# rrrickyz/Parallel-and-Distributed-Deep-Learning

Hardware: AMD Instinct MI355X
Metric: images/sec ResNet-50/ImageNet at 1/2/4/8 MI355X + scaling efficiency (higher is better)
Workload: dtype bf16; 1 GPU; model=ResNet-50 Keras-v1 (25,636,712 params, random init), global_batch=2560, per_gpu_batch=2560, image_size=224, parallelism=dp1, replicas=1, optimizer=adam, bn=frozen (training=False), hip_graph=False, grad_dtype=fp32, device=MI355X

## Files before the change

### csrc/bindings.cpp

```cpp
#include <torch/extension.h>

#include <atomic>
#include <ATen/hip/HIPContext.h>
#include <ATen/hip/impl/HIPGuardImplMasqueradingAsCUDA.h>
#include <c10/util/Optional.h>

#include "kernels/kernels.h"

using torch::Tensor;
using OptT = c10::optional<Tensor>;
namespace py = pybind11;

#define PCHECK(cond, msg) TORCH_CHECK(cond, "pddl: ", msg)

namespace {

std::atomic<bool> g_launched{false};
std::atomic<bool> g_knob_tuning{false};
hipStream_t cur_stream() {
  if (!g_launched.load(std::memory_order_relaxed)) g_launched.store(true, std::memory_order_relaxed);
  return at::hip::getCurrentHIPStream().stream();
}

void ok(const char* err, const char* what) { TORCH_CHECK(err == nullptr, "pddl ", what, ": ", err ? err : ""); }
// ... 744 lines not shown
  m.def("comm_proxy", [](Tensor src, Tensor scratch, int passes, int64_t ticks, int nch) {
    PCHECK(src.is_cuda() && scratch.is_cuda() && src.scalar_type() == torch::kFloat32 &&
               scratch.scalar_type() == torch::kFloat32 && src.is_contiguous() && scratch.is_contiguous() &&
               scratch.numel() >= src.numel() && src.numel() % 4 == 0,
           "comm_proxy: fp32 device tensors, scratch >= src, 4-element multiple");
    ok(pddl::comm_proxy_launch(f32p(src), f32p(scratch), src.numel(), passes, ticks, nch, cur_stream()),
       "comm_proxy");
  }, REL);
  const py::none none;
  m.def("igemm", &igemm, REL, py::arg("a1"), py::arg("a2") = none, py::arg("H"), py::arg("W"), py::arg("R"),
        py::arg("S"), py::arg("stride"), py::arg("pad"), py::arg("Ho"), py::arg("Wo"), py::arg("b"), py::arg("mode"),
        py::arg("scale") = none, py::arg("shift") = none, py::arg("res") = none, py::arg("mask") = none,
        py::arg("add") = none, py::arg("out"), py::arg("relu") = 0, py::arg("out2") = none, py::arg("relu2") = 0,
        py::arg("n_split") = 0, py::arg("up2") = 0, py::arg("Hf") = 0, py::arg("Wf") = 0, py::arg("colsum") = none,
        py::arg("bits_out") = none, py::arg("stats") = none, py::arg("bn_z") = none, py::arg("bn_mean") = none);
  m.def("bn_stats", &bn_stats, REL);
  m.def("bn_apply", &bn_apply, REL, py::arg("z"), py::arg("a"), py::arg("b"), py::arg("r") = none,
        py::arg("a2") = none, py::arg("b2") = none, py::arg("relu"), py::arg("y"), py::arg("bits") = none);
  m.def("bn_bwd_reduce", &bn_bwd_reduce, REL, py::arg("g"), py::arg("z"), py::arg("z2") = none, py::arg("mean"),
        py::arg("mean2") = none, py::arg("sg"), py::arg("sgx"), py::arg("sg2") = none, py::arg("sgx2") = none);
  m.def("bn_bwd_apply", &bn_bwd_apply, REL, py::arg("g"), py::arg("z"), py::arg("z2") = none, py::arg("l"),
        py::arg("l2") = std::vector<double>{}, py::arg("params"), py::arg("mean"), py::arg("inv"), py::arg("sg"),
        py::arg("sgx"), py::arg("dz"), py::arg("dz2") = none, py::arg("grads"), py::arg("coef"));
  m.attr("BNSTAT_LAYER_BYTES") = (int)sizeof(pddl::BnStatLayer);
  m.def("wgrad", &wgrad, REL, py::arg("x"), py::arg("H"), py::arg("W"), py::arg("R"), py::arg("S"),
        py::arg("stride"), py::arg("pad"), py::arg("Ho"), py::arg("Wo"), py::arg("g"), py::arg("g2") = none,
        py::arg("co_split") = 0, py::arg("dw"), py::arg("K"), py::arg("splits") = 0);
  m.def("bwd1x1", &bwd1x1, REL, py::arg("g"), py::arg("x"), py::arg("wd"), py::arg("bits"), py::arg("out"),
        py::arg("colsum"), py::arg("dw"), py::arg("out2") = py::none(), py::arg("g1") = py::none(),
        py::arg("w1d") = py::none(), py::arg("gmask") = py::none(), py::arg("gx") = py::none(),
        py::arg("colsum_gx") = py::none());
  m.def("bwd1x1_partial_rows", &bwd1x1_partial_rows);
  m.def("conv_f32", &conv_f32, REL);
  m.def("conv_f32_epi", &conv_f32_epi, REL, py::arg("x"), py::arg("R"), py::arg("S"), py::arg("stride"),
        py::arg("pad"), py::arg("Ho"), py::arg("Wo"), py::arg("w"), py::arg("epi"), py::arg("scale") = none,
        py::arg("shift") = none, py::arg("res") = none, py::arg("relu") = 0, py::arg("add") = none,
        py::arg("mask") = none, py::arg("up2") = 0, py::arg("y"), py::arg("colsum") = none);
  m.def("maxpool_fwd_f32", &maxpool_fwd_f32, REL);
  m.def("maxpool_bwd_f32", &maxpool_bwd_f32, REL);
  m.def("gap_fwd_f32", &gap_fwd_f32, REL);
  m.def("gap_bwd_f32", &gap_bwd_f32, REL);
  m.def("colsum_f32", &colsum_f32, REL);
  m.def("softmax_xent_f32", &softmax_xent_f32, REL);
  m.def("prep_f32", &prep_f32, REL);
  m.def("wgrad_f32", &wgrad_f32, REL);
  m.def("stem_s2d", &stem_s2d, REL);
  m.def("stem_wgrad_fold", &stem_wgrad_fold, REL);
  m.def("maxpool_fwd", &maxpool_fwd, REL);
  m.def("stem_pool_bwd", &stem_pool_bwd, REL, py::arg("x2"), py::arg("gpool"), py::arg("idx"), py::arg("dw"),
        py::arg("colsum"), py::arg("pool_rows") = 0);
  m.def("stem_pool_bwd_partial_rows", [](int B, int H2, int PB) { return pddl::stem_pool_bwd_partial_rows(B, H2, PB); },
        py::arg("B"), py::arg("H2"), py::arg("pool_rows") = 0);
  m.def("stem_pool_fwd", &stem_pool_fwd, REL, py::arg("x2"), py::arg("w"), py::arg("scale"), py::arg("shift"),
        py::arg("pool"), py::arg("idx"), py::arg("bits") = py::none(), py::arg("pool_rows") = 0);
  m.def("maxpool_bwd", &maxpool_bwd, REL);
  m.def("conv3x3c64", &conv3x3c64, REL, py::arg("x"), py::arg("w"), py::arg("mode"), py::arg("out"),
        py::arg("scale") = py::none(), py::arg("shift") = py::none(), py::arg("bits") = py::none(),
        py::arg("colsum") = py::none());
  m.def("conv3x3c64_wgrad", &conv3x3c64_wgrad, REL, py::arg("x"), py::arg("g"), py::arg("dw"));
  m.def("c3c1", &c3c1, REL, py::arg("a"), py::arg("w3"), py::arg("scale3"), py::arg("shift3"),
        py::arg("res"), py::arg("out"), py::arg("bits3"), py::arg("w1"), py::arg("scale1"), py::arg("shift1"),
        py::arg("y1"), py::arg("bits1"));
  m.def("conv3x3c64_partial_rows", [](int64_t M) { return pddl::conv3x3c64_partial_rows((int)M); });
  m.def("gap_fwd", &gap_fwd, REL);
  m.def("gap_bwd", &gap_bwd, REL);
  m.def("colsum", &colsum, REL);
  m.def("softmax_xent", &softmax_xent, REL);
  m.def("eval_metrics", &eval_metrics, REL);
  m.def("colsum_reduce", &colsum_reduce, REL);
  m.def("allow_knob_changes", [](bool on) { g_knob_tuning.store(on); }, py::arg("on") = true);
  m.def("knobs_frozen", []() { return g_launched.load() && !g_knob_tuning.load(); });
  m.def("set_variant", [](const std::string& which, int v) {
    TORCH_CHECK(!g_launched.load() || g_knob_tuning.load(), "kernel knob ", which,
                ": knobs are read-only once a kernel has launched (set them before the first launch, "
                "e.g. PDDL_KNOBS, or call allow_knob_changes(True) in tuning code)");
    if (which == "igemm") pddl::g_igemm_variant = v;
    else if (which == "igemm_deep") pddl::g_igemm_deep = v;
    else if (which == "igemm_pf") pddl::g_igemm_pf = v;
    else if (which == "igemm8") pddl::g_igemm8 = v;
    else if (which == "igemm8_min_tiles") pddl::g_igemm8_min_tiles = v;
    else if (which == "wgrad8") pddl::g_wgrad8 = v;
    else if (which == "igemm_ns1_kt") pddl::g_igemm_ns1_kt = v;
    else if (which == "igemm8_min_n") pddl::g_igemm8_min_n = v;
    else if (which == "wgrad1") pddl::g_wgrad1 = v;
    else if (which == "igemm_n64") pddl::g_igemm_n64 = v;
    else if (which == "igemm_splitk") pddl::g_igemm_splitk = v;
    else if (which == "igemm_sk_fill") { TORCH_CHECK(v >= 1 && v <= 8, "igemm_sk_fill: 1-8"); pddl::g_igemm_sk_fill = v; }
    else if (which == "igemm_sk_cap") { TORCH_CHECK(v >= 2 && v <= 16, "igemm_sk_cap: 2-16"); pddl::g_igemm_sk_cap = v; }
    else if (which == "igemm_sk_elig") { TORCH_CHECK(v >= 1 && v <= 8, "igemm_sk_elig: 1-8"); pddl::g_igemm_sk_elig = v; }
    else if (which == "igemm_pk_all") pddl::g_igemm_pk_all = v;
    else if (which == "igemm_pk_dual") pddl::g_igemm_pk_dual = v;
    else if (which == "igemm_pk") { TORCH_CHECK(v == 0 || (v >= 2 && v <= 4), "igemm_pk: 0 or ring depth 2-4"); pddl::g_igemm_pk = v; }
    else if (which == "wgrad8_min_rows") { TORCH_CHECK(v >= 64, "wgrad8_min_rows"); pddl::g_wgrad8_min_rows = v; }
    else if (which == "stem") pddl::g_stem_variant = v;
    else if (which == "conv_f32") pddl::g_conv_f32_variant = v;
    else if (which == "conv_f32_splitk") pddl::g_conv_f32_splitk = v;
    else if (which == "conv_f32_sk_elig") { TORCH_CHECK(v >= 1 && v <= 8, "conv_f32_sk_elig: 1-8"); pddl::g_conv_f32_sk_elig = v; }
    else if (which == "wgrad_f32_wpc64") { TORCH_CHECK(v >= 1 && v <= 32, "wgrad_f32_wpc64"); pddl::g_wgrad_f32_wpc[0] = v; }
    else if (which == "wgrad_f32_wpc128") { TORCH_CHECK(v >= 1 && v <= 32, "wgrad_f32_wpc128"); pddl::g_wgrad_f32_wpc[1] = v; }
    else if (which == "c64_grid") pddl::g_c64_grid = v;
    else if (which == "c64w_grid") pddl::g_c64w_grid = v;
    else if (which == "bn_red_blocks") pddl::g_bn_red_blocks = v;
    else if (which == "bn_apply_blocks") pddl::g_bn_apply_blocks = v;
    else if (which == "pool_blocks") pddl::g_pool_blocks = v;
    else if (which == "colred_chunks") { TORCH_CHECK(v >= 1 && v <= 65535, "colred_chunks"); pddl::g_colred_chunks = v; }
    else TORCH_CHECK(false, "unknown kernel knob ", which);
  });
  m.def("wgrad_last_tiling", []() { return pddl::g_wgrad_last_tiling; });
  m.def("stream_capture_deps", [](int64_t stream) {
    hipStreamCaptureStatus st = hipStreamCaptureStatusNone;
    unsigned long long id = 0;
    hipGraph_t g = nullptr;
    const hipGraphNode_t* deps = nullptr;
    size_t n = 0;
    const hipError_t e = hipStreamGetCaptureInfo_v2(reinterpret_cast<hipStream_t>(stream), &st, &id, &g, &deps, &n);
    return std::make_tuple((int)e, (int)st, (int64_t)n);
  });
  m.def("igemm_partial_rows", [](int M, int Nn, int K, bool bnz) { return pddl::igemm_partial_rows(M, Nn, K, bnz); },
        py::arg("M"), py::arg("Nn"), py::arg("K"), py::arg("bnz") = false);
  m.def("igemm_splitk_floats", [](int M, int Nn, int K) { return (int64_t)pddl::igemm_splitk_floats(M, Nn, K); });
  m.def("splitk_use", &splitk_use, py::arg("workspace"));
  m.def("splitk_default_floats", &splitk_default_floats, py::arg("device"));
  m.def("igemm_plan", [](int M, int Nn, int K) {
    int cfg = 0, split = 0, ks = 1;
    pddl::igemm_plan_query(M, Nn, K, &cfg, &split, &ks);
    return std::make_tuple(cfg, split, ks);
  });
  m.def("maxpool_bwd_partial_rows", &pddl::maxpool_bwd_partial_rows);
  m.attr("COLRED_LAYER_BYTES") = (int)sizeof(pddl::ColRedLayer);
  m.def("prep", &prep, REL, py::arg("params"), py::arg("table"), py::arg("nlayers"), py::arg("max_elems"),
        py::arg("wbf"), py::arg("scale"), py::arg("shift"), py::arg("eps"), py::arg("parts") = 3);
  m.def("prep_fuse", &prep_fuse, REL);
  m.def("wgrad_finalize", &wgrad_finalize, REL, py::arg("params"), py::arg("grads"), py::arg("table"),
        py::arg("nlayers"), py::arg("scale"), py::arg("dgamma_raw"), py::arg("max_cout") = 2048);
  m.def("bn_grad", &bn_grad, REL);
  m.def("synth", &synth, REL);
  m.def("opt_hparams", &opt_hparams, REL);
  m.def("adam", &adam, REL);
  m.def("sgd", &sgd, REL);
  m.def("scale_", &scale_, REL);
  m.def("cast_bf16", &cast_bf16, REL);
  m.def("cast_f32", &cast_f32, REL);
  m.attr("PREP_LAYER_BYTES") = (int)sizeof(pddl::PrepLayer);
  m.attr("FUSE_LAYER_BYTES") = (int)sizeof(pddl::FuseLayer);
  m.attr("FIN_LAYER_BYTES") = (int)sizeof(pddl::FinLayer);
  m.attr("BNGRAD_LAYER_BYTES") = (int)sizeof(pddl::BnGradLayer);
  m.attr("EPI_FWD") = (int)pddl::EPI_FWD;
  m.attr("EPI_DGRAD") = (int)pddl::EPI_DGRAD;
  m.attr("EPI_F32") = (int)pddl::EPI_F32;
}
```

### csrc/kernels/igemm.hip

```cpp
#include "common.h"
#include "kernels.h"

namespace pddl {

enum { AM_DIRECT = 0, AM_HALO = 1, AM_DUAL = 2 };

#ifndef IGEMM_MIN_BLOCKS
#define IGEMM_MIN_BLOCKS 2
#endif

__device__ __forceinline__ int sw_chunk(int lane, int i) { return (lane & 7) ^ ((4 * (i & 1) + (lane >> 4)) & 7); }
__device__ __forceinline__ int sw_read(int lane, int kh) { return (((kh * 4) + (lane >> 4)) ^ ((lane >> 1) & 7)) * 16; }

__device__ __forceinline__ uint32_t halo_taps(const IgemmParams& p, int hi, int wi) {
  if (p.R == 3 && p.S == 3) {
    const uint32_t cols = ((unsigned)wi < (unsigned)p.W ? 1u : 0u) | ((unsigned)(wi + 1) < (unsigned)p.W ? 2u : 0u) |
                          ((unsigned)(wi + 2) < (unsigned)p.W ? 4u : 0u);
    return ((unsigned)hi < (unsigned)p.H ? cols : 0u) | ((unsigned)(hi + 1) < (unsigned)p.H ? cols << 3 : 0u) |
           ((unsigned)(hi + 2) < (unsigned)p.H ? cols << 6 : 0u);
  }
  uint32_t rows = 0, cols = 0, mk = 0;
  for (int r = 0; r < p.R; ++r) rows |= (uint32_t)((unsigned)(hi + r) < (unsigned)p.H) << r;
  for (int s = 0; s < p.S; ++s) cols |= (uint32_t)((unsigned)(wi + s) < (unsigned)p.W) << s;
  for (int r = 0; r < p.R; ++r) mk |= ((rows >> r) & 1u) ? cols << (r * p.S) : 0u;
// ... 675 lines not shown
    for (int it = 0; it < 8; ++it) {
      const int row = wm * 64 + it * 8 + (lane >> 3), c = wn * 8 + (lane & 7);
      ra2[it] = (uint32_t)(uintptr_t)LDS_PTR(op_w + row * 256 + ((c ^ pk_sw(row)) << 4));
    }
    v4u_t so[8];
    asm volatile("ds_read_b128 %0, %8\n\tds_read_b128 %1, %9\n\tds_read_b128 %2, %10\n\tds_read_b128 %3, %11\n\t"
                 "ds_read_b128 %4, %12\n\tds_read_b128 %5, %13\n\tds_read_b128 %6, %14\n\tds_read_b128 %7, %15\n\t"
                 "s_waitcnt lgkmcnt(0)"
                 : "=&v"(so[0]), "=&v"(so[1]), "=&v"(so[2]), "=&v"(so[3]), "=&v"(so[4]), "=&v"(so[5]), "=&v"(so[6]),
                   "=&v"(so[7])
                 : "v"(ra2[0]), "v"(ra2[1]), "v"(ra2[2]), "v"(ra2[3]), "v"(ra2[4]), "v"(ra2[5]), "v"(ra2[6]), "v"(ra2[7])
                 : "memory");
#pragma unroll
    for (int it = 0; it < 8; ++it) {
      const int row = wm * 64 + it * 8 + (lane >> 3), c = wn * 8 + (lane & 7);
      const int gc = n0 + c * 8;
      const bool ok = m0 + row < p.M && gc < p.Nn;
      __builtin_amdgcn_raw_buffer_store_b128(so[it], rout, ok ? (uint32_t)((row * p.ldo + gc) * 2) : OOB_OFF, 0, 0);
      if (bits_out)
        __builtin_amdgcn_raw_buffer_store_b8((unsigned char)pos_bits8(make_uint4(so[it].x, so[it].y, so[it].z, so[it].w)), rbo,
                                             ok ? (uint32_t)(row * p.ld_bits_out + (gc >> 3)) : OOB_OFF, 0, 0);
    }
    if (csum_on) {
#pragma unroll
      for (int o = 1; o < 8; o <<= 1)
#pragma unroll
        for (int e = 0; e < 8; ++e) csum[e] += __shfl_xor(csum[e], o, 64);
      const int prow = p.prow_begin + ((m0 - p.m_begin) / BM) * (BM / 64) + wm;
      const __amdgpu_buffer_rsrc_t rcs = __builtin_amdgcn_make_buffer_rsrc(p.colsum + (long)prow * p.Nn, (short)0,
                                                                           p.Nn * 4, 0x00020000);
      const bool w_ok = r8 == 0 && col_ok;
      typedef float v4fl __attribute__((ext_vector_type(4)));
      const v4fl c0 = {csum[0], csum[1], csum[2], csum[3]}, c1 = {csum[4], csum[5], csum[6], csum[7]};
      __builtin_amdgcn_raw_buffer_store_b128(__builtin_bit_cast(v4u_t, c0), rcs, w_ok ? (uint32_t)(gn * 4) : OOB_OFF, 0, 0);
      __builtin_amdgcn_raw_buffer_store_b128(__builtin_bit_cast(v4u_t, c1), rcs, w_ok ? (uint32_t)(gn * 4 + 16) : OOB_OFF,
                                             0, 0);
    }
  }
  asm volatile("s_waitcnt vmcnt(0)" ::: "memory");
}

template <int BM, int BN>
__global__ void __launch_bounds__(256) igemm_splitk_reduce_kernel(IgemmParams p) {
  constexpr int NW = 4, WTM = 64, WTN = 64, TM = 4, TN = 4, WAVES_N = BN / WTN, F = TM * TN;
  constexpr int EPI_LD = 16 + 4;
  __shared__ __attribute__((aligned(16))) float smem[4][32 * EPI_LD];
  const int lane = threadIdx.x & 63;
  const int jw = __builtin_amdgcn_readfirstlane(threadIdx.x >> 6);
  const int sub = blockIdx.x % NW;
  const int wm = sub / WAVES_N, wn = sub % WAVES_N;
  const int nt = (p.Nn + BN - 1) / BN;
  const int tile = blockIdx.x / NW, tn = tile % nt, tm = tile / nt;
  v4f acc[TM][1];
#pragma unroll
  for (int i = 0; i < TM; ++i) acc[i][0] = v4f{0.f, 0.f, 0.f, 0.f};
  const float4* src = reinterpret_cast<const float4*>(p.slab) + ((long)tile * p.ksplit * NW + sub) * F * 64 + jw * 64 + lane;
  const long sstride = (long)NW * F * 64;
  auto add = [&](const float4 (&v)[TM]) {
#pragma unroll
    for (int i = 0; i < TM; ++i) {
      acc[i][0][0] += v[i].x; acc[i][0][1] += v[i].y; acc[i][0][2] += v[i].z; acc[i][0][3] += v[i].w;
    }
  };
  int sl = 0;
  for (; sl + 3 < p.ksplit; sl += 4) {
    float4 v[4][TM];
#pragma unroll
    for (int u = 0; u < 4; ++u)
#pragma unroll
      for (int i = 0; i < TM; ++i) v[u][i] = src[(sl + u) * sstride + i * TN * 64];
#pragma unroll
    for (int u = 0; u < 4; ++u) add(v[u]);
  }
  for (; sl < p.ksplit; ++sl) {
    float4 v[TM];
#pragma unroll
    for (int i = 0; i < TM; ++i) v[i] = src[sl * sstride + i * TN * 64];
    add(v);
  }
  igemm_epilogue<TM, 1, false>(p, acc, p.m_begin + tm * BM + wm * WTM, tn * BN + wn * WTN + jw * 16,
                               p.prow_begin + tm * (BM / WTM) + wm, smem[jw], lane);
}

template <int AM, bool STAGGER>
__global__ void __launch_bounds__(512, 1) igemm8_kernel(IgemmParams p) {
  constexpr int BM = 256, BN = 256, HALF = 16384, BUF = 4 * HALF, LEAD = 5;
  __shared__ __attribute__((aligned(16))) char smem[2 * BUF];
  const int tid = threadIdx.x, lane = tid & 63;
  const int wave = __builtin_amdgcn_readfirstlane(tid >> 6);
  const int wm = wave >> 2, wn = wave & 3;
  const int mt = (p.M - p.m_begin + BM - 1) / BM, nt = (p.Nn + BN - 1) / BN;
  const int wg = xcd_remap(blockIdx.x, mt * nt);
  const int tn = wg % nt, tm = wg / nt;
  const int m0 = p.m_begin + tm * BM, n0 = tn * BN;
  const int HoWo = p.Ho * p.Wo;
  const int n_first = fdiv(m0, p.mg_howo);
  const long HW = (long)p.H * p.W, pix0 = n_first * HW, pix_end = p.N * HW;
  const __amdgpu_buffer_rsrc_t ra1 = make_rsrc_at(p.a1, pix0 * p.C1, pix_end * p.C1);
  const int C2r = AM == AM_DUAL ? p.C2 : p.C1;
  const long HW2 = AM == AM_DUAL ? (long)p.H2 * p.W2 : HW;
  const __amdgpu_buffer_rsrc_t ra2 =
      make_rsrc_at(AM == AM_DUAL ? p.a2 : p.a1, n_first * HW2 * C2r, p.N * HW2 * C2r);
  const __amdgpu_buffer_rsrc_t rb = make_rsrc(p.b, p.Nn * p.ldb * 2);

  uint32_t a_o1[4], a_o2[4], a_taps[4], b_o[4];
#pragma unroll
  for (int hi = 0; hi < 4; ++hi) {
    const int r = 128 * (hi >> 1) + (2 * wave + (hi & 1)) * 8 + (lane >> 3);
    const int m = m0 + r;
    a_o1[hi] = OOB_OFF; a_o2[hi] = OOB_OFF; a_taps[hi] = 0;
    if (m < p.M) {
      const int n = fdiv(m, p.mg_howo), rem = m - n * HoWo;
      const int ho = fdiv(rem, p.mg_wo), wo = rem - ho * p.Wo;
      const int hi_ = ho * p.stride - p.pad, wi = wo * p.stride - p.pad;
      const int pix = ((n - n_first) * p.H + hi_) * p.W + wi;
      a_o1[hi] = (uint32_t)((pix * p.C1 + sw_chunk(lane, hi) * 8) * 2);
      if (AM == AM_DUAL) {
        const int pix2 = ((n - n_first) * p.H2 + ho * p.stride2) * p.W2 + wo * p.stride2;
        a_o2[hi] = (uint32_t)((pix2 * p.C2 + sw_chunk(lane, hi) * 8) * 2);
      }
      if (AM == AM_HALO) a_taps[hi] = halo_taps(p, hi_, wi);
    }
    const int n = n0 + r;
    b_o[hi] = (n < p.Nn) ? (uint32_t)((n * p.ldb + sw_chunk(lane, hi) * 8) * 2) : OOB_OFF;
  }

  int ld_r = 0, ld_s = 0, ld_c0 = 0, ld_src2 = 0, ld_k = 0;
  auto tile_delta = [&]() { return ((ld_r * p.W + ld_s) * (ld_src2 ? p.C2 : p.C1) + ld_c0) * 2; };
  auto advance = [&]() {
    const int C = ld_src2 ? p.C2 : p.C1;
    ld_k += 64;
    ld_c0 += 64;
    if (ld_c0 == C) {
      ld_c0 = 0;
      if (++ld_s == p.S) { ld_s = 0; ++ld_r; }
    }
    if (AM == AM_DUAL && !ld_src2 && ld_k == p.K1) { ld_src2 = 1; ld_r = ld_s = ld_c0 = 0; }
  };
  const int KT = p.K / 64;
  const int NH = 4 * KT;
  auto stage_half = [&](int j, int part) {
    char* base = smem + ((j >> 2) & 1) * BUF;
    const int delta = tile_delta();
    if (part == 0 || part == 3) {
      const int h = part == 0 ? 0 : 1;
      char* hb = base + (part == 0 ? 0 : 3) * HALF;
#pragma unroll
      for (int i = 0; i < 2; ++i) {
        auto dst = LDS_PTR(hb + (2 * wave + i) * 1024);
        const int hi = 2 * h + i;
        if (AM == AM_HALO) {
          const int tap = ld_r * p.S + ld_s;
          const uint32_t off = ((a_taps[hi] >> tap) & 1u) ? a_o1[hi] + (uint32_t)delta : OOB_OFF;
          buf_lds16(ra1, dst, off, 0);
        } else if (AM == AM_DUAL && ld_src2) {
          buf_lds16(ra2, dst, a_o2[hi], delta);
        } else {
          buf_lds16(ra1, dst, a_o1[hi], delta);
        }
      }
    } else {
      const int h = part == 1 ? 0 : 1;
      char* hb = base + part * HALF;
#pragma unroll
      for (int i = 0; i < 2; ++i) buf_lds16(rb, LDS_PTR(hb + (2 * wave + i) * 1024), b_o[2 * h + i], ld_k * 2);
    }
    if (part == 3) advance();
  };
#define IG8_WAIT_BARRIER(need, last)                                                              \
  {                                                                                               \
    const int after_ = (last) - (need);                                                           \
    if (after_ >= 3) asm volatile("s_waitcnt vmcnt(6)\n\ts_barrier" ::: "memory");                \
    else if (after_ == 2) asm volatile("s_waitcnt vmcnt(4)\n\ts_barrier" ::: "memory");           \
    else if (after_ == 1) asm volatile("s_waitcnt vmcnt(2)\n\ts_barrier" ::: "memory");           \
    else asm volatile("s_waitcnt vmcnt(0)\n\ts_barrier" ::: "memory");                            \
  }

  v4f acc[2][2][4][2];
#pragma unroll
  for (int a = 0; a < 2; ++a)
#pragma unroll
    for (int b = 0; b < 2; ++b)
#pragma unroll
      for (int i = 0; i < 4; ++i)
#pragma unroll
        for (int j = 0; j < 2; ++j) acc[a][b][i][j] = v4f{0.f, 0.f, 0.f, 0.f};

#pragma unroll
  for (int j = 0; j < LEAD; ++j)
    if (j < NH) stage_half(j, j & 3);
  {
    const int last = (LEAD < NH ? LEAD : NH) - 1;
    IG8_WAIT_BARRIER(1, last)
  }
  if (STAGGER && wm == 1) asm volatile("s_barrier" ::: "memory");

  v8bf af[2][4], bfr[2][2];
  const int a_row = (wm * 64 + (lane & 15)) * 128;
  const int b_row = (wn * 32 + (lane & 15)) * 128;
  int pos[2];
#pragma unroll
  for (int kh = 0; kh < 2; ++kh) pos[kh] = sw_read(lane, kh);

  for (int t = 0; t < KT; ++t) {
    const char* buf = smem + (t & 1) * BUF;
#pragma unroll
    for (int q = 0; q < 4; ++q) {
      const int qm = (q == 0 || q == 1) ? 0 : 1;
      const int qn = (q == 0 || q == 3) ? 0 : 1;
      const bool loadA = (q == 0 || q == 2), loadB = (q != 2);
      if (loadB) {
        const char* Bs = buf + (qn == 0 ? 1 : 2) * HALF + b_row;
#pragma unroll
        for (int kh = 0; kh < 2; ++kh)
#pragma unroll
          for (int j = 0; j < 2; ++j) bfr[kh][j] = *reinterpret_cast<const v8bf*>(Bs + j * 16 * 128 + pos[kh]);
      }
      __builtin_amdgcn_sched_barrier(0);
      if (loadA) {
        const char* As = buf + (qm == 0 ? 0 : 3) * HALF + a_row;
#pragma unroll
        for (int kh = 0; kh < 2; ++kh)
#pragma unroll
          for (int i = 0; i < 4; ++i) af[kh][i] = *reinterpret_cast<const v8bf*>(As + i * 16 * 128 + pos[kh]);
      }
      const int js = 4 * t + q + LEAD;
      if (js < NH) stage_half(js, (q + LEAD) & 3);
      const int last = (js < NH ? js : NH - 1);
      if (q == 0) IG8_WAIT_BARRIER(4 * t + 2, last)
      else if (q == 1) IG8_WAIT_BARRIER(4 * t + 3, last)
      else if (q == 3 && t + 1 < KT) IG8_WAIT_BARRIER(4 * t + 5, last)
      else asm volatile("s_barrier" ::: "memory");
      __builtin_amdgcn_sched_barrier(0);
      __builtin_amdgcn_s_setprio(1);
#pragma unroll
      for (int kh = 0; kh < 2; ++kh)
#pragma unroll
        for (int i = 0; i < 4; ++i)
#pragma unroll
          for (int j = 0; j < 2; ++j)
            acc[qm][qn][i][j] = __builtin_amdgcn_mfma_f32_16x16x32_bf16(af[kh][i], bfr[kh][j], acc[qm][qn][i][j], 0, 0, 0);
      __builtin_amdgcn_s_setprio(0);
      __builtin_amdgcn_sched_barrier(0);
      asm volatile("s_barrier" ::: "memory");
    }
  }
#undef IG8_WAIT_BARRIER
  if (STAGGER && wm == 0) asm volatile("s_barrier" ::: "memory");
  asm volatile("s_waitcnt vmcnt(0) lgkmcnt(0)" ::: "memory");
  __syncthreads();

  float* stage = reinterpret_cast<float*>(smem) + wave * (32 * (32 + 4));
  const int pr = p.prow_begin + tm * 4;
  igemm_epilogue<4, 2, false>(p, acc[0][0], m0 + wm * 64, n0 + wn * 32, pr + wm, stage, lane);
  igemm_epilogue<4, 2, false>(p, acc[0][1], m0 + wm * 64, n0 + 128 + wn * 32, pr + wm, stage, lane);
  igemm_epilogue<4, 2, false>(p, acc[1][0], m0 + 128 + wm * 64, n0 + wn * 32, pr + 2 + wm, stage, lane);
  igemm_epilogue<4, 2, false>(p, acc[1][1], m0 + 128 + wm * 64, n0 + 128 + wn * 32, pr + 2 + wm, stage, lane);
}

int g_igemm_variant = 0;
int g_igemm_deep = 2;
int g_igemm_pf = 1;
int g_igemm8 = 2;
int g_igemm_ns1_kt = 1000;
int g_igemm8_min_n = 512;
int g_igemm8_min_tiles = 128;
int g_igemm_n64 = 1;

static bool igemm_no_halo(const IgemmParams& p) {
  return p.pad == 0 && (p.Ho - 1) * p.stride + p.R <= p.H && (p.Wo - 1) * p.stride + p.S <= p.W;
}

static bool igemm_check(const IgemmParams& p, const char** why) {
  if (p.K % 64 || p.K1 % 64) { *why = "K must be a multiple of 64"; return false; }
  const bool window = (p.C1 * p.S == 64) && p.stride == 1 && p.pad == 0 && !p.a2;
  if ((p.C1 % 64 && !window) || (p.a2 && p.C2 % 64)) { *why = "channels must be multiples of 64"; return false; }
  if (p.a2 && (p.K - p.K1) % 64) { *why = "second source K must be a multiple of 64"; return false; }
  if (p.a2 && !igemm_no_halo(p)) { *why = "two A sources need an unpadded (1x1) gather"; return false; }
  if (!igemm_no_halo(p) && p.R * p.S > 32) { *why = "padded convs support at most 32 taps"; return false; }
  if (p.Nn % 8 || p.ldb % 8 || p.ldo % 8) { *why = "N / ldb / ldo must be multiples of 8"; return false; }
  if (p.M <= 0 || p.Nn <= 0 || p.K <= 0) { *why = "empty problem"; return false; }
  if (p.bn_z && (p.mode != EPI_DGRAD || p.a2 || p.up2 || !p.stats)) {
    *why = "bn_z: fused BN-backward sums need a single-source dgrad without scatter, with stats rows"; return false;
  }
  if ((long)p.M * p.Ho * p.Wo >= (1L << 40)) { *why = "too many output rows for the magic-number row decode"; return false; }
  const long span = 256 / (p.Ho * p.Wo) + 2, cmax = p.C1 > p.C2 ? p.C1 : p.C2;
  const long hwmax = (long)p.H * p.W > (long)p.H2 * p.W2 ? (long)p.H * p.W : (long)p.H2 * p.W2;
  if (p.a2 && ((p.Ho - 1) * p.stride2 >= p.H2 || (p.Wo - 1) * p.stride2 >= p.W2 || p.stride2 < 1)) {
    *why = "second source geometry does not cover the output rows"; return false;
  }
  if (span * hwmax * cmax * 2 >= (1L << 31) || (long)p.Nn * p.ldb * 2 >= (1L << 31)) {
    *why = "operand too large for 31-bit buffer offsets"; return false;
  }
  if ((long)p.N * hwmax * cmax >= (1L << 31) || (long)p.M * (p.ldo > p.Nn ? p.ldo : p.Nn) >= (1L << 31)) {
    *why = "tensor has more than 2^31 elements"; return false;
  }
  return true;
}

static int igemm_config(int M, int Nn, int K) {
  if (Nn <= 64) return 0;
  if (g_igemm_n64 == 1 && Nn % 128 && Nn % 64 == 0) return 0;
  if (g_igemm_n64 == 2 && K <= 64 && Nn % 64 == 0) return 0;
  if (g_igemm8 && Nn >= g_igemm8_min_n && K >= 256 && Nn < 4 * K && Nn % 256 == 0 &&
      (long)((M + 255) / 256) * ((Nn + 255) / 256) >= g_igemm8_min_tiles)
    return 4;
  return 1;
}
static int igemm_bm(int cfg) { return cfg == 1 ? 128 : 256; }

static int igemm_rows_of(int cfg, int m) {
  const int BM = igemm_bm(cfg);
  return ((m + BM - 1) / BM) * (BM / 64);
}

int num_cus() {
  static int cached[64] = {0};
  int dev = 0;
  if (hipGetDevice(&dev) != hipSuccess || dev < 0 || dev >= 64) return 256;
  if (!cached[dev]) {
    int n = 0;
    if (hipDeviceGetAttribute(&n, hipDeviceAttributeMultiprocessorCount, dev) != hipSuccess || n <= 0) n = 256;
    cached[dev] = n;
  }
  return cached[dev];
}

struct IgemmPlan { int cfg, split, ks; };

int g_igemm_splitk = 1;
int g_igemm_sk_fill = 2, g_igemm_sk_cap = 8, g_igemm_sk_elig = 2;
int g_igemm_pk = 2;
int g_igemm_pk_all = 0;

static int igemm_splitk_slices(int M, int Nn, int K, int cfg) {
  if (!g_igemm_splitk || (cfg != 0 && cfg != 1)) return 1;
  const int KT = K / 64;
  const int BM = igemm_bm(cfg), BN = cfg == 0 ? 64 : 128;
  const long T = (long)((M + BM - 1) / BM) * ((Nn + BN - 1) / BN);
  if (g_igemm_splitk >= 2) return KT >= 2 ? (g_igemm_splitk < KT ? g_igemm_splitk : KT) : 1;
  const long C = num_cus();
  const long target = (long)g_igemm_sk_fill * C;
  if (KT < 8) return 1;
  if ((long)g_igemm_sk_elig * T > C && !(T < target && KT >= 32)) return 1;
  long ks = (target + T - 1) / T;
  if (ks > KT / 4) ks = KT / 4;
  if (ks > g_igemm_sk_cap) ks = g_igemm_sk_cap;
  return ks >= 2 ? (int)ks : 1;
}

static IgemmPlan igemm_plan(int M, int Nn, int K, bool bnz = false) {
  IgemmPlan pl{igemm_config(M, Nn, K), M, 1};
  if (bnz) {
    if (pl.cfg != 0) pl.cfg = 1;
    return pl;
  }
  {
    const int c = pl.cfg == 4 ? 1 : pl.cfg;
    const int ks = igemm_splitk_slices(M, Nn, K, c);
    if (ks > 1) {
      pl.cfg = c;
      pl.ks = ks;
      return pl;
    }
  }
  if (pl.cfg != 4) return pl;
  const int nt = (Nn + 255) / 256, mt = (M + 255) / 256;
  const long T = (long)mt * nt, C = num_cus();
  const long F = T / C, r = T % C;
  if (r == 0 || 2 * r > C) return pl;
  if (F == 0) { pl.cfg = 1; return pl; }
  const long full_m_tiles = (F * C) / nt;
  pl.split = (int)lmin((long)M, full_m_tiles * 256);
  return pl;
}

void igemm_plan_query(int M, int Nn, int K, int* cfg, int* split, int* ksplit) {
  const IgemmPlan pl = igemm_plan(M, Nn, K);
  *cfg = pl.cfg;
  *split = pl.split;
  if (ksplit) *ksplit = pl.ks;
}

long igemm_splitk_floats(int M, int Nn, int K) {
  const IgemmPlan pl = igemm_plan(M, Nn, K);
  if (pl.ks <= 1) return 0;
  const int BM = igemm_bm(pl.cfg), BN = pl.cfg == 0 ? 64 : 128;
  return (long)((M + BM - 1) / BM) * ((Nn + BN - 1) / BN) * pl.ks * BM * BN;
}

int igemm_partial_rows(int M, int Nn, int K, bool bnz) {
  const IgemmPlan pl = igemm_plan(M, Nn, K, bnz);
  return igemm_rows_of(pl.cfg, pl.split) + (pl.split < M ? igemm_rows_of(1, M - pl.split) : 0);
}

static void igemm_launch_cfg(const IgemmParams& p, int cfg, hipStream_t stream);

int g_igemm_pk_dual = 2;
static bool igemm_pk_dual_launch(const IgemmParams& p, hipStream_t stream) {
  const int KT = p.K / 64;
  if (!g_igemm_pk_dual || KT > g_igemm_pk_dual || g_igemm_pk != 2) return false;
  if (p.mode != EPI_FWD || !p.scale || !p.shift || p.res || p.up2 || p.out2 || p.stats || p.bn_z) return false;
  if (p.R != 1 || p.S != 1 || p.pad != 0 || p.C1 != p.K1 || p.C2 != p.K - p.K1 || !igemm_no_halo(p)) return false;
  if (p.Nn % 32) return false;
  const long T = (long)((p.M - p.m_begin + 127) / 128) * ((p.Nn + 127) / 128);
  long G = (long)num_cus() * 2;
  if (G > T) G = T;
#define PKD_GO(KT_) hipLaunchKernelGGL((igemm_pk_kernel<KT_, 2, true, true, true>), dim3((unsigned)G), dim3(256), 0, stream, p)
  if (KT == 2) PKD_GO(2);
  else if (KT == 6) PKD_GO(6);
  else if (KT == 12) PKD_GO(12);
  else if (KT == 24) PKD_GO(24);
  else return false;
#undef PKD_GO
  return true;
}

static bool igemm_pk_launch(const IgemmParams& p, hipStream_t stream) {
  const int KT = p.K / 64;
  if (p.a2) return igemm_pk_dual_launch(p, stream);
  if (p.R != 1 || p.S != 1 || p.pad != 0 || p.C1 != p.K || !igemm_no_halo(p)) return false;
  if (KT != 1 && KT != 2 && KT != 4 && KT != 8) return false;
  if (p.mode != EPI_FWD && p.mode != EPI_DGRAD) return false;
  if (p.up2 || p.out2 || p.stats || p.bn_z || p.mask || p.Nn % 32) return false;
  if (p.mode == EPI_FWD && (!p.scale || !p.shift)) return false;
  const bool ops = p.mode == EPI_FWD || p.add || p.bits_mask;
  if (!ops) return false;
  if (!g_igemm_pk_all && !((p.mode == EPI_DGRAD && p.add) || (p.mode == EPI_FWD && p.res && KT >= 2))) return false;
  const long T = (long)((p.M - p.m_begin + 127) / 128) * ((p.Nn + 127) / 128);
  const int nb = g_igemm_pk;
  long G = (long)num_cus() * (nb == 2 ? 2 : 1);
  if (G > T) G = T;
#define PK_GO(KT_, NB_)                                                                                      \
  {                                                                                                          \
    if (p.mode == EPI_FWD) hipLaunchKernelGGL((igemm_pk_kernel<KT_, NB_, true, true>), dim3((unsigned)G), dim3(256), 0, stream, p); \
    else hipLaunchKernelGGL((igemm_pk_kernel<KT_, NB_, true, false>), dim3((unsigned)G), dim3(256), 0, stream, p); \
  }
#define PK_NB(KT_)                          \
  {                                         \
    if (nb == 2) PK_GO(KT_, 2)              \
    else if (nb == 3) PK_GO(KT_, 3)         \
    else PK_GO(KT_, 4)                      \
  }
  if (KT == 1) PK_NB(1) else if (KT == 2) PK_NB(2) else if (KT == 4) PK_NB(4) else PK_NB(8)
#undef PK_NB
#undef PK_GO
  return true;
}

const char* igemm_launch(const IgemmParams& p_in, hipStream_t stream) {
  const char* why = nullptr;
  if (!igemm_check(p_in, &why)) return why;
  IgemmParams p = p_in;
  p.mg_howo = fdiv_magic(p.Ho * p.Wo);
  p.mg_wo = fdiv_magic(p.Wo);
  p.m_begin = 0;
  p.prow_begin = 0;
  p.ksplit = 1;
  const IgemmPlan pl = igemm_plan(p.M, p.Nn, p.K, p.bn_z != nullptr);
  if (g_igemm_pk && pl.ks == 1 && ((pl.split >= p.M && pl.cfg == 1) || p.a2) && igemm_pk_launch(p, stream)) {
    hipError_t e = hipGetLastError();
    return e == hipSuccess ? nullptr : hipGetErrorString(e);
  }
  const bool window = (p.C1 * p.S == 64) && p.C1 < 64;
  if (pl.ks > 1 && !p.a2 && !window && p.C1 % 64 == 0 && p.slab && !(p.mode == EPI_FWD && p.up2) &&
      p.slab_floats >= igemm_splitk_floats(p.M, p.Nn, p.K)) {
    p.ksplit = pl.ks;
    const int BM = igemm_bm(pl.cfg), BN = pl.cfg == 0 ? 64 : 128;
    const int tiles = ((p.M + BM - 1) / BM) * ((p.Nn + BN - 1) / BN);
    igemm_launch_cfg(p, pl.cfg, stream);
    if (pl.cfg == 0) hipLaunchKernelGGL((igemm_splitk_reduce_kernel<256, 64>), dim3(tiles * 4), dim3(256), 0, stream, p);
    else hipLaunchKernelGGL((igemm_splitk_reduce_kernel<128, 128>), dim3(tiles * 4), dim3(256), 0, stream, p);
  } else if (pl.split < p.M) {
    IgemmParams head = p, tail = p;
    head.M = pl.split;
    tail.m_begin = pl.split;
    tail.prow_begin = igemm_rows_of(pl.cfg, pl.split);
    igemm_launch_cfg(head, pl.cfg, stream);
    igemm_launch_cfg(tail, 1, stream);
  } else {
    igemm_launch_cfg(p, pl.cfg, stream);
  }
  hipError_t e = hipGetLastError();
  return e == hipSuccess ? nullptr : hipGetErrorString(e);
}

static void igemm_launch_cfg(const IgemmParams& p, int cfg, hipStream_t stream) {
  const int KT = p.K / 64;
  int ns = g_igemm_variant;
  if (ns == 0) ns = KT <= g_igemm_ns1_kt ? 1 : 2;
  const int am = p.a2 ? AM_DUAL : (igemm_no_halo(p) ? AM_DIRECT : AM_HALO);
#define IG_GO(BM_, BN_, NS_, AM_) \
  hipLaunchKernelGGL((igemm_kernel<BM_, BN_, NS_, AM_>), dim3(nwg), dim3(256), 0, stream, p)
#define IG_MODES(BM_, BN_, NS_)                                 \
  {                                                             \
    if (am == AM_DIRECT) IG_GO(BM_, BN_, NS_, AM_DIRECT);       \
    else if (am == AM_HALO) IG_GO(BM_, BN_, NS_, AM_HALO);      \
    else IG_GO(BM_, BN_, NS_, AM_DUAL);                         \
  }
  const int BM = igemm_bm(cfg), BN = cfg == 0 ? 64 : (cfg == 4 ? 256 : 128);
  const int nwg = ((p.M - p.m_begin + BM - 1) / BM) * ((p.Nn + BN - 1) / BN) * (p.ksplit > 1 ? p.ksplit : 1);
  if (p.ksplit > 1) {
#define IG_SK(BM_, BN_, NS_, AM_) \
  hipLaunchKernelGGL((igemm_kernel<BM_, BN_, NS_, AM_, false, false, true>), dim3(nwg), dim3(256), 0, stream, p)
    if (cfg == 1) {
      if (ns == 1) { if (am == AM_DIRECT) IG_SK(128, 128, 1, AM_DIRECT); else IG_SK(128, 128, 1, AM_HALO); }
      else { if (am == AM_DIRECT) IG_SK(128, 128, 2, AM_DIRECT); else IG_SK(128, 128, 2, AM_HALO); }
    } else {
      if (ns == 1) { if (am == AM_DIRECT) IG_SK(256, 64, 1, AM_DIRECT); else IG_SK(256, 64, 1, AM_HALO); }
      else { if (am == AM_DIRECT) IG_SK(256, 64, 2, AM_DIRECT); else IG_SK(256, 64, 2, AM_HALO); }
    }
#undef IG_SK
    return;
  }
  const bool pf = g_igemm_pf && am == AM_DIRECT && cfg <= 1 &&
                  ((p.mode == EPI_FWD && p.res) || (p.mode == EPI_DGRAD && p.add && !p.up2 && (ns == 2 || g_igemm_pf == 2)));
  if (p.bn_z) {
#define IG_Z(BM_, BN_, AM_) \
  hipLaunchKernelGGL((igemm_kernel<BM_, BN_, 1, AM_, false, true>), dim3(nwg), dim3(256), 0, stream, p)
    if (cfg == 0) {
      if (am == AM_DIRECT) IG_Z(256, 64, AM_DIRECT); else IG_Z(256, 64, AM_HALO);
    } else {
      if (am == AM_DIRECT) IG_Z(128, 128, AM_DIRECT); else IG_Z(128, 128, AM_HALO);
    }
#undef IG_Z
  } else if (cfg == 4) {
#define IG_8(AM_)                                                                                         \
  {                                                                                                       \
    if (g_igemm8 == 2) hipLaunchKernelGGL((igemm8_kernel<AM_, true>), dim3(nwg), dim3(512), 0, stream, p); \
    else hipLaunchKernelGGL((igemm8_kernel<AM_, false>), dim3(nwg), dim3(512), 0, stream, p);             \
  }
    if (am == AM_DIRECT) IG_8(AM_DIRECT)
    else if (am == AM_HALO) IG_8(AM_HALO)
    else IG_8(AM_DUAL)
#undef IG_8
  } else if (pf) {
#define IG_PF(BM_, BN_, NS_) \
  hipLaunchKernelGGL((igemm_kernel<BM_, BN_, NS_, AM_DIRECT, true>), dim3(nwg), dim3(256), 0, stream, p)
    if (cfg == 1) {
      if (ns == 1) IG_PF(128, 128, 1); else IG_PF(128, 128, 2);
    } else {
      if (ns == 1) IG_PF(256, 64, 1); else IG_PF(256, 64, 2);
// ... 13 lines not shown
```

### csrc/kernels/kernels.h

```cpp
#pragma once
#include <hip/hip_runtime.h>
#include <stdint.h>

namespace pddl {

enum EpiMode { EPI_FWD = 0, EPI_DGRAD = 1, EPI_F32 = 2 };

struct IgemmParams {
  const uint16_t* a1; int C1;
  const uint16_t* a2; int C2;
  int H2, W2, stride2;
  int N, H, W;
  int R, S, stride, pad;
  int Ho, Wo, M;
  int K1, K;
  const uint16_t* b; int ldb; int Nn;
  int mode;
  const float* scale; const float* shift;
  const uint16_t* res; int ld_res;
  const uint16_t* mask; int ld_mask;
  const uint16_t* add; int ld_add;
  void* out; int ldo; int relu;
  void* out2; int ldo2; int relu2; int n_split;
  int up2; int Hf, Wf;
  float* colsum;
  uint8_t* bits_out; int ld_bits_out;
  const uint8_t* bits_mask; int ld_bits_mask;
  float* stats;
  const uint16_t* bn_z; const float* bn_mean;
  uint64_t mg_howo, mg_wo;
  int m_begin, prow_begin;
  float* slab; long slab_floats;
  int ksplit;
};
const char* igemm_launch(const IgemmParams& p, hipStream_t stream);
int igemm_partial_rows(int M, int Nn, int K, bool bnz = false);
void igemm_plan_query(int M, int Nn, int K, int* cfg, int* split, int* ksplit = nullptr);
long igemm_splitk_floats(int M, int Nn, int K);
extern int g_igemm8, g_igemm8_min_tiles, g_igemm8_min_n, g_igemm_ns1_kt, g_wgrad8, g_wgrad1;
int num_cus();
extern int g_wgrad_f32_wpc[2];
extern int g_wgrad_last_tiling;
extern int g_igemm_sk_fill, g_igemm_sk_cap, g_igemm_sk_elig;
extern int g_igemm_splitk, g_wgrad8_min_rows, g_igemm_pk, g_igemm_pk_all, g_igemm_pk_dual;
extern int g_stem_variant, g_igemm_n64, g_igemm_variant, g_igemm_deep, g_igemm_pf, g_bn_red_blocks, g_bn_apply_blocks, g_pool_blocks, g_colred_chunks;

struct WgradParams {
  const uint16_t* x; int N, H, W, C;
  int ldx;
  int R, S, stride, pad, Ho, Wo, M;
  const uint16_t* g; int ldg;
  const uint16_t* g2; int ldg2; int co_split;
  int Cout, K;
  float* dw; int ld_dw;
  int splits;
};
const char* wgrad_launch(const WgradParams& p, hipStream_t stream);

struct Bwd1x1Params {
  const uint16_t* g;
  const uint16_t* x;
  const uint16_t* wd; int ld_wd;
  const uint8_t* bits;
  uint16_t* out;
  float* colsum;
  float* dw; int ld_dw;
  int M, CO, CI;
  int s2, N, Hf, Wf, Hc, Wc;
  uint16_t* out2;
  uint64_t mg_hwc, mg_wc;
  const uint16_t* g1;
  const uint16_t* w1d;
  const uint8_t* gmask;
  uint16_t* gx;
  float* colsum_gx;
};
const char* bwd1x1_launch(const Bwd1x1Params& p, hipStream_t stream);
int bwd1x1_partial_rows(int M, int CO, int CI);

struct ConvF32Params {
  const float* x; int N, H, W, C;
  int R, S, stride, pad, Ho, Wo, M;
  const float* w; const float* bias;
  int Cout, K;
  float* y;
  float* dw;
  uint64_t mg_howo, mg_wo;
  int epi;
  const float* scale; const float* shift; const float* res; int relu;
  const float* add; const float* mask; int up2, Hf, Wf;
  float* colsum;
  float* slab; long slab_floats;
  int ksplit;
};
enum { F32_EPI_PLAIN = 0, F32_EPI_FWD = 1, F32_EPI_DGRAD = 2 };
const char* conv_f32_launch(ConvF32Params p, hipStream_t stream);
extern int g_conv_f32_variant, g_conv_f32_splitk, g_conv_f32_sk_elig;
const char* wgrad_f32_launch(ConvF32Params p, hipStream_t stream);
const char* maxpool_fwd_f32_launch(const float* x, float* y, uint8_t* idx, int B, int H, int W, int C, int Ho, int Wo,
                                   hipStream_t s);
const char* maxpool_bwd_f32_launch(const float* gy, const uint8_t* idx, const float* xmask, float* gx, int B, int H,
                                   int W, int C, int Ho, int Wo, hipStream_t s);
const char* gap_fwd_f32_launch(const float* x, float* y, int B, int HW, int C, hipStream_t s);
const char* gap_bwd_f32_launch(const float* gp, const float* ymask, float* g, int B, int HW, int C, float* colsum_rows,
                               hipStream_t s);
const char* colsum_f32_launch(const float* g, long M, int C, int ldg, float* out, hipStream_t s);
const char* softmax_xent_f32_launch(const float* logits, int ldl, const int64_t* labels, int B, int ncls, float gscale,
                                    float* dlogits, int ldd, float* loss_sum, float* correct, hipStream_t s);

struct StemParams {
  const void* in; int in_u8;
  int B, Hin, Win;
  int Hc, Wc;
  int mode;
  int oy, ox;
  const int32_t* crop_dev;
  const uint8_t* flip;
  float scale;
  uint16_t* out; int Hs, Ws;
};
const char* stem_s2d_launch(const StemParams& p, hipStream_t s);
const char* stem_s2d_f32_launch(const StemParams& p, float* out, hipStream_t s);
// ... 182 lines not shown
```

Measured before the change: 31360 images/sec.

## Software-pipeline LDS fragment reads in igemm8 and widen its eligibility to N=256

Restructures the 256x256 igemm8 main loop so the LDS fragment reads for the next quadrant are issued between MFMAs of the current quadrant. It double-buffers the A/B register fragments, uses immediate-offset ds_read_b128 and finer vmcnt waits, so LDS latency is hidden behind matrix math instead of stalling before each quadrant. It also lets forward/plain GEMMs with N=256, large K and many tiles (no row-stat epilogues) use the 8-wave kernel, via a new tunable threshold. This raises register pressure, and the hand-placed waitcnt/barrier scheduling is fragile.

```diff
diff --git a/csrc/bindings.cpp b/csrc/bindings.cpp
--- a/csrc/bindings.cpp
+++ b/csrc/bindings.cpp
@@ -850,6 +850,7 @@
     else if (which == "wgrad8") pddl::g_wgrad8 = v;
     else if (which == "igemm_ns1_kt") pddl::g_igemm_ns1_kt = v;
     else if (which == "igemm8_min_n") pddl::g_igemm8_min_n = v;
+    else if (which == "igemm8_n256_min_k") pddl::g_igemm8_n256_min_k = v;
     else if (which == "wgrad1") pddl::g_wgrad1 = v;
     else if (which == "igemm_n64") pddl::g_igemm_n64 = v;
     else if (which == "igemm_splitk") pddl::g_igemm_splitk = v;
@@ -889,11 +890,11 @@
   m.def("igemm_splitk_floats", [](int M, int Nn, int K) { return (int64_t)pddl::igemm_splitk_floats(M, Nn, K); });
   m.def("splitk_use", &splitk_use, py::arg("workspace"));
   m.def("splitk_default_floats", &splitk_default_floats, py::arg("device"));
-  m.def("igemm_plan", [](int M, int Nn, int K) {
+  m.def("igemm_plan", [](int M, int Nn, int K, bool no_rows) {
     int cfg = 0, split = 0, ks = 1;
-    pddl::igemm_plan_query(M, Nn, K, &cfg, &split, &ks);
+    pddl::igemm_plan_query(M, Nn, K, &cfg, &split, &ks, no_rows);
     return std::make_tuple(cfg, split, ks);
-  });
+  }, py::arg("M"), py::arg("Nn"), py::arg("K"), py::arg("no_rows") = false);
   m.def("maxpool_bwd_partial_rows", &pddl::maxpool_bwd_partial_rows);
   m.attr("COLRED_LAYER_BYTES") = (int)sizeof(pddl::ColRedLayer);
   m.def("prep", &prep, REL, py::arg("params"), py::arg("table"), py::arg("nlayers"), py::arg("max_elems"),
diff --git a/csrc/kernels/igemm.hip b/csrc/kernels/igemm.hip
--- a/csrc/kernels/igemm.hip
+++ b/csrc/kernels/igemm.hip
@@ -781,6 +781,14 @@
                                p.prow_begin + tm * (BM / WTM) + wm, smem[jw], lane);
 }
 
+template <int OFF>
+__device__ __forceinline__ v8bf ig8_read_at(uint32_t addr) {
+  static_assert(OFF >= 0 && OFF < 65536, "ds_read immediate offset is 16 bits");
+  v8bf r;
+  asm volatile("ds_read_b128 %0, %1 offset:%2" : "=v"(r) : "v"(addr), "n"(OFF) : "memory");
+  return r;
+}
+
 template <int AM, bool STAGGER>
 __global__ void __launch_bounds__(512, 1) igemm8_kernel(IgemmParams p) {
   constexpr int BM = 256, BN = 256, HALF = 16384, BUF = 4 * HALF, LEAD = 5;
@@ -874,6 +882,12 @@
     else if (after_ == 1) asm volatile("s_waitcnt vmcnt(2)\n\ts_barrier" ::: "memory");           \
     else asm volatile("s_waitcnt vmcnt(0)\n\ts_barrier" ::: "memory");                            \
   }
+#define IG8_WAIT_BARRIER_AT(need, nominal)                                                        \
+  {                                                                                               \
+                     \
+    if (steady) asm volatile("s_waitcnt vmcnt(%0)\n\ts_barrier" :: "n"(2 * ((nominal) - (need)) + 0 * AM) : "memory"); \
+    else IG8_WAIT_BARRIER(need, NH - 1)                                                           \
+  }
 
   v4f acc[2][2][4][2];
 #pragma unroll
@@ -890,61 +904,107 @@
     if (j < NH) stage_half(j, j & 3);
   {
     const int last = (LEAD < NH ? LEAD : NH) - 1;
-    IG8_WAIT_BARRIER(1, last)
+    IG8_WAIT_BARRIER(STAGGER ? 2 : 1, last)
   }
   if (STAGGER && wm == 1) asm volatile("s_barrier" ::: "memory");
 
-  v8bf af[2][4], bfr[2][2];
-  const int a_row = (wm * 64 + (lane & 15)) * 128;
-  const int b_row = (wn * 32 + (lane & 15)) * 128;
-  int pos[2];
-#pragma unroll
-  for (int kh = 0; kh < 2; ++kh) pos[kh] = sw_read(lane, kh);
-
-  for (int t = 0; t < KT; ++t) {
-    const char* buf = smem + (t & 1) * BUF;
-#pragma unroll
-    for (int q = 0; q < 4; ++q) {
-      const int qm = (q == 0 || q == 1) ? 0 : 1;
-      const int qn = (q == 0 || q == 3) ? 0 : 1;
-      const bool loadA = (q == 0 || q == 2), loadB = (q != 2);
-      if (loadB) {
-        const char* Bs = buf + (qn == 0 ? 1 : 2) * HALF + b_row;
+  uint32_t fa[2], fb[2];
+#pragma unroll
+  for (int kh = 0; kh < 2; ++kh) {
+    const uint32_t base = (uint32_t)(uintptr_t)LDS_PTR(smem) + sw_read(lane, kh);
+    fa[kh] = base + (wm * 64 + (lane & 15)) * 128;
+    fb[kh] = base + (wn * 32 + (lane & 15)) * 128;
+  }
+  v8bf af[2][2][4], bfr[2][2][2];
+  uint32_t boff = 0;
+#define IG8_READ_A(d, part, bo, kh, i)                                                            \
+  {                                                                                               \
+    const uint32_t a_ = fa[kh] + (bo);                                                            \
+    d = (i) == 0 ? ig8_read_at<(part) * HALF>(a_) : (i) == 1 ? ig8_read_at<(part) * HALF + 2048>(a_) \
+      : (i) == 2 ? ig8_read_at<(part) * HALF + 4096>(a_) : ig8_read_at<(part) * HALF + 6144>(a_); \
+  }
+#define IG8_READ_B(d, part, bo, kh, j)                                                            \
+  {                                                                                               \
+    const uint32_t a_ = fb[kh] + (bo);                                                            \
+    d = (j) == 0 ? ig8_read_at<(part) * HALF>(a_) : ig8_read_at<(part) * HALF + 2048>(a_);        \
+  }
+#define IG8_LANDED_A(s)                                                                           \
+  asm volatile("s_waitcnt lgkmcnt(0)"                                                             \
+               : "+v"(af[s][0][0]), "+v"(af[s][0][1]), "+v"(af[s][0][2]), "+v"(af[s][0][3]),      \
+                 "+v"(af[s][1][0]), "+v"(af[s][1][1]), "+v"(af[s][1][2]), "+v"(af[s][1][3])       \
+               :: "memory");
+#define IG8_LANDED_B(s)                                                                           \
+  asm volatile("s_waitcnt lgkmcnt(0)"                                                             \
+               : "+v"(bfr[s][0][0]), "+v"(bfr[s][0][1]), "+v"(bfr[s][1][0]), "+v"(bfr[s][1][1])   \
+               :: "memory");
+#pragma unroll
+  for (int kh = 0; kh < 2; ++kh) {
+#pragma unroll
+    for (int j = 0; j < 2; ++j) IG8_READ_B(bfr[0][kh][j], 1, 0u, kh, j)
+#pragma unroll
+    for (int i = 0; i < 4; ++i) IG8_READ_A(af[0][kh][i], 0, 0u, kh, i)
+  }
+  for (int t2 = 0; t2 < KT; t2 += 2) {
+#pragma unroll
+    for (int par = 0; par < 2; ++par) {
+      const int t = t2 + par;
+      if (t >= KT) break;
+      asm volatile("" : "+s"(boff));
+      const uint32_t nboff = boff ^ (uint32_t)BUF;
+      const bool more = t + 1 < KT;
+#pragma unroll
+      for (int q = 0; q < 4; ++q) {
+        const int qm = (q == 0 || q == 1) ? 0 : 1;
+        const int qn = (q == 0 || q == 3) ? 0 : 1;
+        const int xs = qn ^ par;
+        const int js = 4 * t + q + LEAD;
+        const bool steady = js < NH;
+        if (steady) stage_half(js, (q + LEAD) & 3);
+        if (q == 0 || q == 2) IG8_LANDED_A(qm)
+        if (q != 2) IG8_LANDED_B(xs)
+        if (!STAGGER) {
+          if (q == 0) IG8_WAIT_BARRIER_AT(4 * t + 2, js)
+          else if (q == 1) IG8_WAIT_BARRIER_AT(4 * t + 3, js)
+          else if (q == 3 && more) IG8_WAIT_BARRIER_AT(4 * t + 5, js)
+          else asm volatile("s_barrier" ::: "memory");
+        } else {
+          if (q == 0) IG8_WAIT_BARRIER_AT(4 * t + 3, js)
+          else if (q == 2 && more) IG8_WAIT_BARRIER_AT(4 * t + 5, js)
+          else if (q == 3 && more) IG8_WAIT_BARRIER_AT(4 * t + 6, js)
+          else asm volatile("s_barrier" ::: "memory");
+        }
+        __builtin_amdgcn_sched_barrier(0);
+        __builtin_amdgcn_s_setprio(1);
 #pragma unroll
         for (int kh = 0; kh < 2; ++kh)
 #pragma unroll
-          for (int j = 0; j < 2; ++j) bfr[kh][j] = *reinterpret_cast<const v8bf*>(Bs + j * 16 * 128 + pos[kh]);
-      }
-      __builtin_amdgcn_sched_barrier(0);
-      if (loadA) {
-        const char* As = buf + (qm == 0 ? 0 : 3) * HALF + a_row;
-#pragma unroll
-        for (int kh = 0; kh < 2; ++kh)
-#pragma unroll
-          for (int i = 0; i < 4; ++i) af[kh][i] = *reinterpret_cast<const v8bf*>(As + i * 16 * 128 + pos[kh]);
-      }
-      const int js = 4 * t + q + LEAD;
-      if (js < NH) stage_half(js, (q + LEAD) & 3);
-      const int last = (js < NH ? js : NH - 1);
-      if (q == 0) IG8_WAIT_BARRIER(4 * t + 2, last)
-      else if (q == 1) IG8_WAIT_BARRIER(4 * t + 3, last)
-      else if (q == 3 && t + 1 < KT) IG8_WAIT_BARRIER(4 * t + 5, last)
-      else asm volatile("s_barrier" ::: "memory");
-      __builtin_amdgcn_sched_barrier(0);
-      __builtin_amdgcn_s_setprio(1);
-#pragma unroll
-      for (int kh = 0; kh < 2; ++kh)
-#pragma unroll
-        for (int i = 0; i < 4; ++i)
-#pragma unroll
-          for (int j = 0; j < 2; ++j)
-            acc[qm][qn][i][j] = __builtin_amdgcn_mfma_f32_16x16x32_bf16(af[kh][i], bfr[kh][j], acc[qm][qn][i][j], 0, 0, 0);
-      __builtin_amdgcn_s_setprio(0);
-      __builtin_amdgcn_sched_barrier(0);
-      asm volatile("s_barrier" ::: "memory");
-    }
-  }
+          for (int i = 0; i < 4; ++i)
+#pragma unroll
+            for (int j = 0; j < 2; ++j) {
+              acc[qm][qn][i][j] = __builtin_amdgcn_mfma_f32_16x16x32_bf16(af[qm][kh][i], bfr[xs][kh][j], acc[qm][qn][i][j], 0, 0, 0);
+              const int n = (kh * 4 + i) * 2 + j;
+              if (q == 0 && n < 4) IG8_READ_B(bfr[xs ^ 1][n >> 1][n & 1], 2, boff, n >> 1, n & 1)
+              if (q == 1 && n < 8) IG8_READ_A(af[1][n >> 2][n & 3], 3, boff, n >> 2, n & 3)
+              if (q == 2 && n < 4) IG8_READ_B(bfr[xs ^ 1][n >> 1][n & 1], 1, boff, n >> 1, n & 1)
+              if (q == 3 && n < 4) IG8_READ_B(bfr[xs ^ 1][n >> 1][n & 1], 1, nboff, n >> 1, n & 1)
+              if (q == 3 && n >= 4 && n < 12) IG8_READ_A(af[0][(n - 4) >> 2][(n - 4) & 3], 0, nboff, (n - 4) >> 2, (n - 4) & 3)
+              __builtin_amdgcn_sched_barrier(0);
+            }
+        __builtin_amdgcn_s_setprio(0);
+        asm volatile("s_barrier" ::: "memory");
+      }
+      boff = nboff;
+    }
+  }
+  IG8_LANDED_A(0)
+  IG8_LANDED_B(0)
+  IG8_LANDED_B(1)
 #undef IG8_WAIT_BARRIER
+#undef IG8_WAIT_BARRIER_AT
+#undef IG8_READ_A
+#undef IG8_READ_B
+#undef IG8_LANDED_A
+#undef IG8_LANDED_B
   if (STAGGER && wm == 0) asm volatile("s_barrier" ::: "memory");
   asm volatile("s_waitcnt vmcnt(0) lgkmcnt(0)" ::: "memory");
   __syncthreads();
@@ -964,6 +1024,7 @@
 int g_igemm_ns1_kt = 1000;
 int g_igemm8_min_n = 512;
 int g_igemm8_min_tiles = 128;
+int g_igemm8_n256_min_k = 2304;
 int g_igemm_n64 = 1;
 
 static bool igemm_no_halo(const IgemmParams& p) {
@@ -997,12 +1058,15 @@
   return true;
 }
 
-static int igemm_config(int M, int Nn, int K) {
+static int igemm_config(int M, int Nn, int K, bool no_rows = false) {
   if (Nn <= 64) return 0;
   if (g_igemm_n64 == 1 && Nn % 128 && Nn % 64 == 0) return 0;
   if (g_igemm_n64 == 2 && K <= 64 && Nn % 64 == 0) return 0;
-  if (g_igemm8 && Nn >= g_igemm8_min_n && K >= 256 && Nn < 4 * K && Nn % 256 == 0 &&
-      (long)((M + 255) / 256) * ((Nn + 255) / 256) >= g_igemm8_min_tiles)
+  const long tiles8 = (long)((M + 255) / 256) * ((Nn + 255) / 256);
+  const bool wide = Nn >= g_igemm8_min_n ||
+                    (no_rows && Nn >= 256 && K >= g_igemm8_n256_min_k && tiles8 >= 8L * g_igemm8_min_tiles);
+  if (g_igemm8 && wide && K >= 256 && Nn < 4 * K && Nn % 256 == 0 &&
+      tiles8 >= g_igemm8_min_tiles)
     return 4;
   return 1;
 }
@@ -1048,8 +1112,8 @@
   return ks >= 2 ? (int)ks : 1;
 }
 
-static IgemmPlan igemm_plan(int M, int Nn, int K, bool bnz = false) {
-  IgemmPlan pl{igemm_config(M, Nn, K), M, 1};
+static IgemmPlan igemm_plan(int M, int Nn, int K, bool bnz = false, bool no_rows = false) {
+  IgemmPlan pl{igemm_config(M, Nn, K, no_rows && !bnz), M, 1};
   if (bnz) {
     if (pl.cfg != 0) pl.cfg = 1;
     return pl;
@@ -1068,14 +1132,14 @@
   const long T = (long)mt * nt, C = num_cus();
   const long F = T / C, r = T % C;
   if (r == 0 || 2 * r > C) return pl;
-  if (F == 0) { pl.cfg = 1; return pl; }
+  if (F == 0) { if (g_igemm8_min_tiles > 1) pl.cfg = 1; return pl; }
   const long full_m_tiles = (F * C) / nt;
   pl.split = (int)lmin((long)M, full_m_tiles * 256);
   return pl;
 }
 
-void igemm_plan_query(int M, int Nn, int K, int* cfg, int* split, int* ksplit) {
-  const IgemmPlan pl = igemm_plan(M, Nn, K);
+void igemm_plan_query(int M, int Nn, int K, int* cfg, int* split, int* ksplit, bool no_rows) {
+  const IgemmPlan pl = igemm_plan(M, Nn, K, false, no_rows);
   *cfg = pl.cfg;
   *split = pl.split;
   if (ksplit) *ksplit = pl.ks;
@@ -1156,7 +1220,8 @@
   p.m_begin = 0;
   p.prow_begin = 0;
   p.ksplit = 1;
-  const IgemmPlan pl = igemm_plan(p.M, p.Nn, p.K, p.bn_z != nullptr);
+  const bool no_rows = p.mode != EPI_DGRAD && !p.stats && !p.colsum && !p.bn_z;
+  const IgemmPlan pl = igemm_plan(p.M, p.Nn, p.K, p.bn_z != nullptr, no_rows);
   if (g_igemm_pk && pl.ks == 1 && ((pl.split >= p.M && pl.cfg == 1) || p.a2) && igemm_pk_launch(p, stream)) {
     hipError_t e = hipGetLastError();
     return e == hipSuccess ? nullptr : hipGetErrorString(e);
diff --git a/csrc/kernels/kernels.h b/csrc/kernels/kernels.h
--- a/csrc/kernels/kernels.h
+++ b/csrc/kernels/kernels.h
@@ -35,9 +35,9 @@
 };
 const char* igemm_launch(const IgemmParams& p, hipStream_t stream);
 int igemm_partial_rows(int M, int Nn, int K, bool bnz = false);
-void igemm_plan_query(int M, int Nn, int K, int* cfg, int* split, int* ksplit = nullptr);
+void igemm_plan_query(int M, int Nn, int K, int* cfg, int* split, int* ksplit = nullptr, bool no_rows = false);
 long igemm_splitk_floats(int M, int Nn, int K);
-extern int g_igemm8, g_igemm8_min_tiles, g_igemm8_min_n, g_igemm_ns1_kt, g_wgrad8, g_wgrad1;
+extern int g_igemm8, g_igemm8_min_tiles, g_igemm8_min_n, g_igemm8_n256_min_k, g_igemm_ns1_kt, g_wgrad8, g_wgrad1;
 int num_cus();
 extern int g_wgrad_f32_wpc[2];
 extern int g_wgrad_last_tiling;
```

Result: no change. 31520 images/sec, median of 6 (+0.5%).
